# lutao98/SqrtLM-SLAM

Measured on AMD Instinct MI355X. Metric: LM iterations/sec (synthetic KITTI-00-scale BA), higher is better.
Workload: dtype f64; 1 GPU; synthetic global BA (BASELINE config 4); n_pose=5000, n_landmark=500000, n_obs=4999754, track_len=U{2..18}, robust=False, seed=4, parallelism=landmark-shard x1, comm=none, comm_ranks=1

## Files before the change

### include/sqrtlm.h

```cpp
#ifndef SQRTLM_H
#define SQRTLM_H

#include <stdint.h>

#ifdef __cplusplus
extern "C" {
#endif

#define SQLM_OK 0
#define SQLM_ERR_INVALID_ARG (-1)
#define SQLM_ERR_HIP (-2)
#define SQLM_ERR_NOT_SPD (-3)
#define SQLM_ERR_OOM (-4)
#define SQLM_ERR_ABORTED (-5)
#define SQLM_ERR_NO_DEVICE (-6)
#define SQLM_ERR_STATE (-7)
#define SQLM_ERR_UNSUPPORTED (-8)
#define SQLM_ERR_COMM (-9)

#define SQLM_TRACE_MAX 256

typedef struct sqlm_ctx sqlm_ctx;

typedef struct sqlm_stats {
// ... 225 lines not shown
#define SQLM_COMM_RCCL_SELFLOOP 2
#define SQLM_COMM_HOST 3
int sqlm_ctx_comm_info(const sqlm_ctx *ctx, int *transport, int *rank, int *nranks);
int sqlm_ctx_set_comm_selfloop(sqlm_ctx *ctx, const char *unique_id);
int sqlm_comm_selftest(int device, const char *unique_id, int64_t count, double *max_err);

#define SQLM_DT_F64 0
#define SQLM_DT_U8 1
#define SQLM_DT_I32 2
#define SQLM_OP_SUM 0
#define SQLM_OP_MAX 1
typedef int (*sqlm_allreduce_fn)(void *user, void *buf, int64_t count, int dtype, int op);
int sqlm_ctx_set_host_comm(sqlm_ctx *ctx, int rank, int nranks, sqlm_allreduce_fn fn, void *user);
#define SQLM_P2P_SEND 0
#define SQLM_P2P_RECV 1
#define SQLM_P2P_BCAST 2
typedef int (*sqlm_p2p_fn)(void *user, void *buf, int64_t count, int dtype, int peer, int op);
int sqlm_ctx_set_host_p2p(sqlm_ctx *ctx, sqlm_p2p_fn fn, void *user);

#define SQLM_NKERNEL_TIMERS 9
int sqlm_bench_iterations(sqlm_ctx *ctx, int warmup, int n, double *ms_per_iter, double *kernel_ms,
                          sqlm_stats *stats);
const char *sqlm_kernel_timer_name(int i);

#ifdef __cplusplus
}
#endif
#endif
```

### sqrtlm-slam_amd/csrc/sqlm_api.cpp

```cpp
#include <hip/hip_runtime.h>

#include <algorithm>
#include <cmath>
#include <cstring>
#include <new>
#include <vector>

#include "../../include/sqrtlm.h"
#include "../../include/sqrtlm_orb.h"
#include "se3_dev.h"
#include "sqlm_ctx.h"

using namespace sqlm;

namespace {

const char *kTimerNames[SQLM_NKERNEL_TIMERS] = {"k_linearize", "k_camera_pass", "k_damp", "k_rcs_tile",
                                                "k_solve", "k_pose_update", "k_landmark_update", "reduce+sync",
                                                "k_rcs_reduce"};

void depth_positive_host(const sqlm_ctx *c, std::vector<uint8_t> &out) {
  out.resize(c->n_obs);
  for (int64_t e = 0; e < c->n_obs; ++e) {
    const int p = c->obs_pose[e];
// ... 966 lines not shown
  s = comm_barrier(c->comm, c->stream);
  if (s) return s;
  c->timing = kernel_ms != nullptr;
  std::fill(c->kernel_ms_acc, c->kernel_ms_acc + SQLM_NKERNEL_TIMERS, 0.0);
  c->kernel_ms_n = 0;
  Timer t;
  s = run_lm(c, n, 0.0, nullptr, st, nullptr, true);
  SQLM_HIP_OK(hipStreamSynchronize(c->stream));
  const double ms = t.ms();
  c->timing = false;
  if (s) return s;
  if (ms_per_iter) *ms_per_iter = ms / n;
  if (kernel_ms) {
    for (int i = 0; i < SQLM_NKERNEL_TIMERS; ++i)
      kernel_ms[i] = c->kernel_ms_n ? c->kernel_ms_acc[i] / c->kernel_ms_n : 0.0;
  }
  return finish(c);
}

#ifdef SQLM_TILE_PROF
int sqlm_debug_tile_profile(long long *out) { return sqlm::tile_profile_read(out); }
#endif

const char *sqlm_kernel_timer_name(int i) {
  return (i >= 0 && i < SQLM_NKERNEL_TIMERS) ? kTimerNames[i] : "";
}

static int orb_engine(sqlm_ctx *c) {
  if (!c) return SQLM_ERR_INVALID_ARG;
  if (hipSetDevice(c->device) != hipSuccess) return SQLM_ERR_HIP;
  if (!c->orb && !(c->orb = orb_create(c->stream))) return SQLM_ERR_OOM;
  return SQLM_OK;
}

int sqlm_orb_extract(sqlm_ctx *c, const sqlm_orb_params *p, const uint8_t *image, int w, int h, int stride,
                     sqlm_keypoint *kps, uint8_t *desc, int cap, int *n_out) {
  if (int r = orb_engine(c)) return r;
  return orb_extract(c->orb, p, image, w, h, stride, kps, desc, cap, n_out);
}

int sqlm_orb_get_level(sqlm_ctx *c, int level, uint8_t *out, int cap, int *lw, int *lh) {
  if (!c || !c->orb) return SQLM_ERR_STATE;
  if (hipSetDevice(c->device) != hipSuccess) return SQLM_ERR_HIP;
  return orb_get_level(c->orb, level, out, cap, lw, lh);
}

// ... 82 lines not shown
```

### sqrtlm-slam_amd/csrc/sqlm_cr_aug.h

```cpp
#pragma once

namespace sqlm {
namespace aug {

#ifdef SQLM_AUG_SOLO
constexpr bool kPipe = false;
#else
constexpr bool kPipe = true;
#endif

constexpr int kWaves = 16, kThreads = 64 * kWaves, kMaxNt = kCRMaxN / 16, kWorkers = kPipe ? 10 : 12;
constexpr int kPairs = kMaxNt * (kMaxNt - 1) / 2;
enum : int { kNone = 0, kColD = 1, kColI0 = 3, kColEt = 4, kColE = 5, kColG = 6 };

#ifndef SQLM_SPIN_LIMIT
#define SQLM_SPIN_LIMIT (1 << 20)
#endif
constexpr int kSpinLimit = SQLM_SPIN_LIMIT;
constexpr int kTp = 17;
struct Shared {
  double T[kMaxNt][16 * kTp];
  double U[kPairs][256];
  double Hp[kMaxNt][256];
  double Hq[kMaxNt][256];
// ... 287 lines not shown
    if (q == 0) {
      sh.bx[16 * i + r] = x;
      st_d(v.x + (size_t)I * n + 16 * i + r, x);
    }
    __builtin_amdgcn_fence(__ATOMIC_RELEASE, "wavefront");
    __builtin_amdgcn_wave_barrier();
    __builtin_amdgcn_fence(__ATOMIC_ACQUIRE, "wavefront");
  }
}

constexpr int kCrErrTimeout = 1;
__device__ __forceinline__ void cr_fail(const CRView &v, int lane) {
  if (lane == 0) {
    __hip_atomic_store(v.flags, 0, __ATOMIC_RELAXED, __HIP_MEMORY_SCOPE_AGENT);
    __hip_atomic_store(v.flags + 1, kCrErrTimeout, __ATOMIC_RELAXED, __HIP_MEMORY_SCOPE_AGENT);
  }
}

template <int MODE, bool LINV, bool BACK>
__device__ __forceinline__ void aug_body(aug::Shared &sh, const CRView &v, int h, int I, int split, int sidx) {
  using namespace aug;
  const int lane = threadIdx.x & 63, wave = threadIdx.x >> 6;
  const int n = v.n, nt = n >> 4;
  const bool left = MODE == 0, right = MODE != 1 && I + h < v.p, first = sidx == 0;
  bool tmo = false;
  for (int t = threadIdx.x; t < 2 * kMaxNt + kPairs + 17; t += blockDim.x) {
    if (t < kMaxNt) sh.fT[t] = 0;
    else if (t < kMaxNt + kPairs) sh.fU[t - kMaxNt] = 0;
    else if (t < 2 * kMaxNt + kPairs) sh.fH[t - kMaxNt - kPairs] = 0;
    else if (t < 2 * kMaxNt + kPairs + 8) (&sh.fA[0][0])[t - 2 * kMaxNt - kPairs] = 0;
    else if (t < 2 * kMaxNt + kPairs + 16) (&sh.fO[0][0])[t - 2 * kMaxNt - kPairs - 8] = 0;
    else sh.fD = 0;
  }
  __syncthreads();
#ifdef SQLM_SPIN_DEBUG
  if (lane == 0 && (wave == 0 || wave == 9))
    printf("aug blk %d wave %d I %d mode %d past zeroing, fT0 %d\n", (int)blockIdx.x, wave, I, MODE, sh.fT[0]);
#endif
  if (threadIdx.x == 0) AUG_PROF(0);
  AUG_HWID(wave);
  const bool dense = MODE == 1 && v.ld;
  const int ldd = dense ? v.ld : n;
  const double *Dblk = dense ? v.D : blk(v.D, I, n);
  bool bad = false;
  if (kPipe && wave == 0) {
    __builtin_amdgcn_s_setprio(3);
    AUG_PROF(1);
// ... 284 lines not shown
```

### sqrtlm-slam_amd/csrc/sqlm_internal.h

```cpp
#pragma once
#include <hip/hip_runtime.h>
#include <stdint.h>

#include <cfloat>
#include <cmath>
#include <vector>

#include "../../include/sqrtlm.h"

namespace sqlm {

#define SQLM_HIP_OK(x)                          \
  do {                                          \
    if ((x) != hipSuccess) return SQLM_ERR_HIP; \
  } while (0)

#ifndef SQLM_TILE_MAXCAMS
#define SQLM_TILE_MAXCAMS 24
#endif
#ifndef SQLM_TILE_MAXLM
#define SQLM_TILE_MAXLM 128
#endif
constexpr int kTileMaxCams = SQLM_TILE_MAXCAMS, kTileHardCams = 24, kTileMaxLm = SQLM_TILE_MAXLM, kTileMaxK = 1 << 20;
constexpr int kTileNtMax = (6 * kTileHardCams + 15) / 16;
// ... 165 lines not shown
  int *flags = nullptr;
};

enum Scalar { kChiCur = 0, kChiNew = 1, kScale = 2, kMaxDiag = 3, kSolveOk = 4, kDevErr = 5, kNScalars = 8 };
constexpr int kMboxSeq = 7;

enum PartialRegion {
  kPartChiCurLm = 0,
  kPartChiCurLid = 16384,
  kPartChiNewLm = 147456,
  kPartChiNewLid = 163840,
  kPartScaleCam = 180224,
  kPartScaleLm = 196608,
  kPartChiCurLm2 = 212992,
  kPartChiCurLid2 = 229376,
  kPartEnd = 360448
};
constexpr int kMaxPartials = kPartEnd;
constexpr int kMaxFreePoses = 131072;

struct CRPlan {
  bool enabled = false;
  int B = 0, p = 0, n = 0;
  int nband = 0;
  int R = 0, Rp = 0, nbc = 0;
  std::vector<int> sched;
  const int *sched_dev = nullptr;
  std::vector<int> lvl;
  int init_off = 0, init_cnt = 0;
  int elim_off = 0, elim_cnt = 0;
  bool top_active = false;
};
constexpr int kCRMaxN = 112;
constexpr int kBandMaxCams = kCRMaxN / 6 - 1;
constexpr int kUpdHad = 1 << 28, kUpdRight = 1 << 29, kUpdLeft = 1 << 30, kUpdMask = (1 << 28) - 1;

__host__ __device__ inline int tile_blk(int u, int w, int cp) { return u * (2 * cp - u + 1) / 2 + (w - u); }

#ifndef SQLM_OBS_PER_LANE
#define SQLM_OBS_PER_LANE 3
#endif
constexpr int kObsPerLane = SQLM_OBS_PER_LANE;
#ifndef SQLM_OBS_PRELOAD
#define SQLM_OBS_PRELOAD 2
#endif
constexpr int kObsPreload = SQLM_OBS_PRELOAD;
// ... 34 lines not shown
void launch_rcs_tiles(const DevProblem &d, double lambda, hipStream_t st, const TileStreams *ts = nullptr);
enum TileKernel {
  kTileKernelNone = 0,
  kTileKernelRows = 1,
  kTileKernelMono = 2,
  kTileKernelStereo = 3,
  kTileKernelProducer = 4,
};
int rcs_tile_kernel(const DevProblem &d);
void launch_rcs_reduce(const DevProblem &d, double lambda, hipStream_t st);
#ifdef SQLM_TILE_PROF
int tile_profile_read(long long *out);
#endif
constexpr int kRedLong = 24;
int launch_dense_solve(const DevProblem &d, hipStream_t st);
struct CRSync {
  int *done = nullptr;
  int cap = 0, epoch = 0;
};
int launch_cr_solve(const DevProblem &d, const CRPlan &pl, hipStream_t st, bool gather = true,
                    CRSync *sync = nullptr);
void launch_arrow_clear(const DevProblem &d, const CRPlan &pl, hipStream_t st);
void launch_cr_core(double *D, double *L, double *E, double *A, double *C, double *g, double *x, int *flags, int p, int n,
                    hipStream_t st, CRSync *sync = nullptr);
int launch_dense_spd_solve(double *A, double *L, double *Linv, double *r, double *x, int *flags, int n,
                           hipStream_t st, int band = 0, int n_last = 0);
int launch_cr_multi(double *D, double *L, double *E, double *A, double *C, double *gs, double *xs, double *G, double *Z,
                    double *X, int *flags, int p, int n, int R, hipStream_t st);
int launch_batched_atb(const double *A, const double *B, double *P, int p, int n, int R, hipStream_t st);
void launch_pose_update(const DevProblem &d, double lambda, hipStream_t st, bool from_cr = false);
void launch_landmark_update(const DevProblem &d, const Bucket &b, double lambda, int part_off, hipStream_t st,
                            bool spec = false, bool fuse_pose = false);
constexpr int kMaxUpdBuckets = 6;
struct UpdLaunch {
  int nb = 0, grid = 0;
  int W[kMaxUpdBuckets], slot_begin[kMaxUpdBuckets], slot_end[kMaxUpdBuckets], part_off[kMaxUpdBuckets],
      rng_off[kMaxUpdBuckets], nblk[kMaxUpdBuckets], blk0[kMaxUpdBuckets];
};
int upd_launch_plan(const std::vector<Bucket> &bk, const std::vector<int> &part_off, UpdLaunch &u);
void launch_landmark_update_all(const DevProblem &d, const UpdLaunch &u, double lambda, hipStream_t st, bool spec);
void launch_lidar_chi2(const DevProblem &d, hipStream_t st);
void launch_reduce(const DevProblem &d, int n_lm_parts_cur, int n_lm_parts_new, int n_cam_parts,
                   int n_lid_parts, hipStream_t st, double *mbox = nullptr, unsigned long long seq = 0);
void launch_depth_positive(const DevProblem &d, uint8_t *out_dev, hipStream_t st);

int linearize_blocks(const Bucket &b);

// ... 350 lines not shown
```

### sqrtlm-slam_amd/csrc/sqlm_plan.cpp

```cpp
#include "sqlm_plan.h"

#include <limits>
#include <queue>

namespace sqlm {

void build_tiles(int nP, int nL, const std::vector<int> &lm_begin, const int *obs_camh, int lm_cap, TilePlan &tp,
                 TileBuild &tb, int *obs_local) {
  const int64_t nE = lm_begin[nL];
  PhaseTimer sub(kPhaseTiles);
  tp.reset();
  tp.urange.assign(nL, int2{-1, -1});
  std::vector<int> &tstart = tb.tstart;
  tstart.clear();
  {
    const int nchunk = (int)std::max<int64_t>(1, std::min<int64_t>(16, nE / 131072));
    const int nth = std::min(nchunk, host_threads(nE));
    std::vector<std::vector<int>> cuts(nchunk);
    std::vector<uint8_t> dup(nchunk, 0);
    run_threads(nth, [&](int th) {
      std::vector<int> stamp(nP, -1), lmst(nP, -1);
      for (int ch = th; ch < nchunk; ch += nth) {
        const int s0 = (int)((int64_t)nL * ch / nchunk), s1 = (int)((int64_t)nL * (ch + 1) / nchunk);
        std::vector<int> &cv = cuts[ch];
// ... 280 lines not shown
      }
      deg[v] = 0;
    }
  }
  const int nband = nP - nbc;
  if (nbc > 0) {
    if (nband == 0 || 3 * nbc > nP) return false;
    int pos = 0, b = 0;
    for (int i = 0; i < nP; ++i) cam_pos[i] = border[i] ? -1 - b++ : pos++;
  }
  int bw = 0;
  for (int i = 0; i < nP; ++i)
    for (int k = s_row[i]; k < s_row[i + 1]; ++k)
      if (cam_pos[i] >= 0 && cam_pos[s_col[k]] >= 0) bw = std::max(bw, cam_pos[s_col[k]] - cam_pos[i]);
  int B = std::min(bw + 1, std::max(nband, 1));
  if (nbc == 0) B = cr_superblock_width(B, nband);
  const int n = (6 * B + 15) / 16 * 16;
  if (n > kCRMaxN) return false;
  pl.enabled = true;
  pl.B = B;
  pl.p = (nband + B - 1) / B;
  pl.n = n;
  pl.nband = nband;
  if (nbc == 0) return true;
  pl.nbc = nbc;
  pl.R = (6 * nbc + 15) / 16 * 16;
  pl.Rp = (pl.R + kCRMaxN - 1) / kCRMaxN * kCRMaxN;
  std::vector<uint8_t> act(pl.p, 0);
  for (int i = 0; i < nP; ++i)
    for (int k = s_row[i]; k < s_row[i + 1]; ++k) {
      const int a = cam_pos[i], c2 = cam_pos[s_col[k]];
      if ((a < 0) != (c2 < 0)) act[(a >= 0 ? a : c2) / B] = 1;
    }
  std::vector<int> &S = pl.sched, elim;
  pl.init_off = 0;
  for (int I = 0; I < pl.p; ++I)
    if (act[I]) S.push_back(I);
  pl.init_cnt = (int)S.size();
  for (int h = 1; h < pl.p; h *= 2) {
    const int fo = (int)S.size();
    for (int I = h; I < pl.p; I += 2 * h)
      if (act[I]) { S.push_back(I); elim.push_back(I); }
    const int uo = (int)S.size();
    for (int J = 0; J < pl.p; J += 2 * h) {
      const bool r = J + h < pl.p && act[J + h], l = J >= h && act[J - h];
      if (!r && !l) continue;
      S.push_back(J | (act[J] ? kUpdHad : 0) | (r ? kUpdRight : 0) | (l ? kUpdLeft : 0));
// ... 508 lines not shown
```

### sqrtlm-slam_amd/csrc/sqlm_plan.h

```cpp
#pragma once
#include <cstdint>
#include <vector>

#include "sqlm_host_par.h"
#include "sqlm_internal.h"

namespace sqlm {

struct TilePlan {
  std::vector<int> lm_ptr{0}, cam_ptr{0}, cams, ld, red_ptr, gred_ptr;
  std::vector<int2> urange, gred_idx;
  std::vector<int64_t> red_off;
  std::vector<int64_t> gred_off;
  std::vector<int> long_s, long_g;
  std::vector<int64_t> part_ptr{0}, gpart_ptr{0};
  int max_cp = 0;
  bool dups = false;
  std::vector<int> order;
  int cls_off[kTileNtMax + 2] = {}, cls_cnt[kTileNtMax + 1] = {};
  void reset() {
    lm_ptr.assign(1, 0);
    cam_ptr.assign(1, 0);
    part_ptr.assign(1, 0);
    gpart_ptr.assign(1, 0);
// ... 2 lines not shown
    gred_idx.clear();
    red_off.clear();
    gred_off.clear();
    max_cp = 0;
    dups = false;
    std::fill(cls_off, cls_off + kTileNtMax + 2, 0);
    std::fill(cls_cnt, cls_cnt + kTileNtMax + 1, 0);
  }
};

struct TileBuild {
  struct Red { int key, tile, code, j; };
  struct TileOut { std::vector<int> cams; std::vector<Red> red; };
  std::vector<int> tstart;
  std::vector<TileOut> out;
};

void build_tiles(int nP, int nL, const std::vector<int> &lm_begin, const int *obs_camh, int lm_cap, TilePlan &tp,
                 TileBuild &tb, int *obs_local);
void pattern_from_tiles(int nP, const TileBuild &tb, std::vector<int> &s_row, std::vector<int> &s_col);
void build_tiles_finish(int nP, const std::vector<int> &s_row, const std::vector<int> &s_col, TilePlan &tp,
                        TileBuild &tb);
int cr_superblock_width(int bmin, int nband);
bool plan_rcs(int nP, const std::vector<int> &s_row, const std::vector<int> &s_col, CRPlan &pl,
              std::vector<int> &cam_pos);

inline int seg_width(int k) {
  int w = 2;
  while (kObsPerLane * w < k && w < 64) w <<= 1;
  return w;
}

struct GraphView {
  int n_pose = 0, n_pt = 0;
  int64_t n_obs = 0, n_lid = 0;
  const int32_t *obs_pose = nullptr, *obs_pt = nullptr;
  const double *obs_uv = nullptr, *obs_info = nullptr, *obs_delta = nullptr;
  const uint8_t *obs_level = nullptr;
  const double *obs_ur = nullptr;
  const uint8_t *pose_fixed = nullptr;
  const int32_t *lid_pose = nullptr;
  const double *lid_pc = nullptr, *lid_pw = nullptr, *lid_n = nullptr, *lid_info = nullptr;
  const uint8_t *lid_level = nullptr;
  const uint8_t *lid_kind = nullptr;
  int level = 0;
};
// ... 58 lines not shown
```

### sqrtlm-slam_amd/csrc/sqlm_rcs_solve.hip

```cpp
#include <hip/hip_runtime.h>

#include <algorithm>
#include <climits>
#include <cstdlib>

#include "sqlm_internal.h"

namespace sqlm {

typedef double d4 __attribute__((ext_vector_type(4)));

__device__ __forceinline__ void st_d(double *p, double v) { *p = v; }

#ifdef SQLM_CR_PROF
__device__ long long *g_cr_prof;
#define CR_PROF(i)                                                                    \
  do {                                                                                \
    if (threadIdx.x == 0 && g_cr_prof) g_cr_prof[blockIdx.x * 64 + (i)] = clock64(); \
  } while (0)
#else
#define CR_PROF(i) \
  do {             \
  } while (0)
#endif

__device__ __forceinline__ double readlane_d(double v, int l) {
  const int lo = __builtin_amdgcn_readlane(__double2loint(v), l);
  const int hi = __builtin_amdgcn_readlane(__double2hiint(v), l);
  return __hiloint2double(hi, lo);
// ... 233 lines not shown
        const int k = 4 * s + k4;
        a[4 * t + s] = t > jb ? L[(16 * jb + k) * ld + 16 * t + r16] : Dinv[jb * kTile + k * kT + r16];
        b[4 * t + s] = z[16 * t + k];
      }
    }
  double acc = 0.0;
#pragma unroll
  for (int t = 0; t < kCRMaxN / 16; ++t)
    if (t >= jb && t < nt) {
#pragma unroll
      for (int s = 0; s < 4; ++s) acc = fma(a[4 * t + s], b[4 * t + s], acc);
    }
  return k4_sum(acc);
}

struct CRView {
  int p, n, B, nP;
  double *D, *E, *A, *C, *g, *x;
  int *flags;
  double *L;
  int ld;
  int *done = nullptr;
  int epoch = 0;
};

__device__ __forceinline__ double *blk(double *base, int I, int n) { return base + (size_t)I * n * n; }

inline size_t cr_factor_lds(int n) { return ((size_t)n * (n + 1) + 37 * (size_t)n) * sizeof(double); }

__global__ __launch_bounds__(256) void k_cr_scatter(DevProblem d, CRView v) {
  const int i = blockIdx.x;
  const int n = v.n, R = d.arw_R, Rp = d.arw_Rp;
  const int pi = d.cam_pos ? d.cam_pos[i] : i;
  const int I = pi >= 0 ? pi / v.B : 0, li = pi >= 0 ? pi - I * v.B : 0;
  for (int s = d.s_row_ptr[i]; s < d.s_row_ptr[i + 1]; ++s) {
    const int j = d.s_col[s];
    const int pj = d.cam_pos ? d.cam_pos[j] : j;
    const int J = pj >= 0 ? pj / v.B : 0, lj = pj >= 0 ? pj - J * v.B : 0;
    for (int e = threadIdx.x; e < 36; e += blockDim.x) {
      const int r = e / 6, c = e % 6;
      const double val = d.S[(size_t)s * 36 + e];
      if (pi >= 0 && pj >= 0) {
        if (J == I) {
          blk(v.D, I, n)[(6 * li + r) * n + 6 * lj + c] = val;
          if (j != i) blk(v.D, I, n)[(6 * lj + c) * n + 6 * li + r] = val;
        } else {
// ... 212 lines not shown
  const int jobs = (I + h < v.p ? 2 : 1) * nt;
  const int q0 = sidx + split * wave, q1 = sidx + split * (wave + nw);
  double b0x[kCRMaxN / 8], b0y[kCRMaxN / 8], b1x[kCRMaxN / 8], b1y[kCRMaxN / 8];
  if (sidx == 0) cr_factor_store(v, I, lds, &fail);
  else cr_factor_block(v, I, lds, &fail);
  const double *L = lds, *Dinv = lds + n * ld + 2 * n;
  if (q0 < jobs) {
    if (q0 < nt) load_strip<true>(blk(v.E, I - h, n), n, q0, b0x, b0y);
    else load_strip<false>(blk(v.E, I, n), n, q0 - nt, b0x, b0y);
  }
  if (q1 < jobs) {
    if (q1 < nt) load_strip<true>(blk(v.E, I - h, n), n, q1, b1x, b1y);
    else load_strip<false>(blk(v.E, I, n), n, q1 - nt, b1x, b1y);
  }
  if (q0 < jobs) strip_tiles(L, ld, Dinv, b0x, b0y, q0 < nt ? blk(v.A, I, n) : blk(v.C, I, n), n, q0 % nt);
  if (q1 < jobs) strip_tiles(L, ld, Dinv, b1x, b1y, q1 < nt ? blk(v.A, I, n) : blk(v.C, I, n), n, q1 % nt);
}

inline int cr_split(int n_odd, int nt) { return std::max(1, std::min(2 * nt, 256 / std::max(1, n_odd))); }

__device__ __forceinline__ void cr_update_item(const CRView &v, int h, int lb) {
  const int n = v.n, nt = n >> 4, nd = nt * (nt + 1) / 2, items = nd + nt * nt + nt;
  const int ev = lb / items, rem = lb - ev * items;
  const int J = 2 * h * ev;
  const bool right = J + h < v.p, left = J >= h;
  const int lane = threadIdx.x & 63, r16 = lane & 15, k4 = lane >> 4;
  if (rem < nd) {
    int ti = 0, tj = rem;
    while (tj > ti) { tj -= ti + 1; ++ti; }
    d4 acc = {0.0, 0.0, 0.0, 0.0};
    if (right) acc = tile_gemm<true, false, false>(blk(v.A, J + h, n), blk(v.A, J + h, n), n, ti, tj);
    if (left) {
      const d4 a2 = tile_gemm<true, false, false>(blk(v.C, J - h, n), blk(v.C, J - h, n), n, ti, tj);
      acc += a2;
    }
    if (right || left) tile_store(blk(v.D, J, n), n, ti, tj, acc, -1.0, true);
  } else if (rem < nd + nt * nt) {
    const int t = rem - nd, ti = t / nt, tj = t - ti * nt;
    if (right && J + 2 * h < v.p) {
      const d4 acc = tile_gemm<true, false, false>(blk(v.A, J + h, n), blk(v.C, J + h, n), n, ti, tj);
      tile_store(blk(v.E, J, n), n, ti, tj, acc, -1.0, false);
    }
  } else {
    const int ar = 16 * (rem - nd - nt * nt) + r16;
    double s = 0.0;
    if (right) {
      const double *A = blk(v.A, J + h, n), *z = v.g + (size_t)(J + h) * n;
#pragma unroll
      for (int u = 0; u < kCRMaxN / 4; ++u) {
        const int k = kclamp(4 * u + k4, n);
        s += A[k * n + ar] * (4 * u < n ? z[k] : 0.0);
      }
    }
    if (left) {
      const double *C = blk(v.C, J - h, n), *z = v.g + (size_t)(J - h) * n;
#pragma unroll
      for (int u = 0; u < kCRMaxN / 4; ++u) {
        const int k = kclamp(4 * u + k4, n);
        s += C[k * n + ar] * (4 * u < n ? z[k] : 0.0);
      }
    }
    s = k4_sum(s);
// ... 17 lines not shown
  if (wave < nt) {
    const double s = linv_gemv(L, ld, Dinv, tmp, wave);
    if (k4 == 0) z[ar] = s;
  }
  __syncthreads();
  if (wave < nt) {
    const double s = linv_gemv_t(L, ld, Dinv, z, wave, nt);
    if (k4 == 0) v.x[ar] = s;
  }
  CR_PROF(34);
}

__global__ __launch_bounds__(512) void k_cr_top(CRView v) {
  extern __shared__ __attribute__((aligned(16))) double lds[];
  __shared__ int fail;
  cr_top_body(v, lds, &fail);
}

template <bool LINV>
__device__ __forceinline__ void cr_back_body(const CRView &v, int h, int I, double *t) {
  const int n = v.n;
  const int wave = threadIdx.x >> 6, lane = threadIdx.x & 63, lo = lane & 7, hi = lane >> 3;
  const bool act = wave < (n >> 4);
  const bool right = I + h < v.p;
  using d2 = HIP_vector_type<double, 2>;
  const int ca = 2 * lo;
  const d2 *A = reinterpret_cast<const d2 *>(blk(v.A, I, n)), *C = reinterpret_cast<const d2 *>(blk(v.C, I, n));
  const d2 *xl = reinterpret_cast<const d2 *>(v.x + (size_t)(I - h) * n);
  const d2 *xr = reinterpret_cast<const d2 *>(v.x + (size_t)(I + (right ? h : 0)) * n);
  const d2 *Li = reinterpret_cast<const d2 *>(blk(v.L, I, n));
  const int r0 = 16 * wave + hi, hn = n >> 1;
  d2 a0[kCRMaxN / 16], a1[kCRMaxN / 16], c0[kCRMaxN / 16], c1[kCRMaxN / 16], vl[kCRMaxN / 16], vr[kCRMaxN / 16];
  d2 li[kCRMaxN / 8];
  if (act) {
#pragma unroll
  for (int u = 0; u < kCRMaxN / 16; ++u) {
    const int c = kclamp(16 * u + ca, n) >> 1;
    a0[u] = A[r0 * hn + c];
    a1[u] = A[(r0 + 8) * hn + c];
    vl[u] = xl[c];
  }
  if (LINV) {
#pragma unroll
    for (int u = 0; u < kCRMaxN / 8; ++u) li[u] = Li[kclamp(16 * wave + 8 * u + hi, n) * hn + 8 * wave + lo];
  }
  if (right) {
#pragma unroll
    for (int u = 0; u < kCRMaxN / 16; ++u) {
      const int c = kclamp(16 * u + ca, n) >> 1;
      c0[u] = C[r0 * hn + c];
      c1[u] = C[(r0 + 8) * hn + c];
      vr[u] = xr[c];
    }
  }
  double s0 = 0.0, s1 = 0.0;
#pragma unroll
  for (int u = 0; u < kCRMaxN / 16; ++u)
    if (16 * u < n) {
      s0 += a0[u].x * vl[u].x + a0[u].y * vl[u].y;
      s1 += a1[u].x * vl[u].x + a1[u].y * vl[u].y;
      if (right) {
        s0 += c0[u].x * vr[u].x + c0[u].y * vr[u].y;
        s1 += c1[u].x * vr[u].x + c1[u].y * vr[u].y;
// ... 71 lines not shown
    }
  acc += __shfl_xor(acc, 16, 64);
  acc += __shfl_xor(acc, 32, 64);
  if (q == 0) rr[16 * i + r] = y[16 * i + r] - acc;
  __builtin_amdgcn_fence(__ATOMIC_RELEASE, "wavefront");
  __builtin_amdgcn_wave_barrier();
  __builtin_amdgcn_fence(__ATOMIC_ACQUIRE, "wavefront");
  double x = 0.0;
#pragma unroll
  for (int m = 0; m < 4; ++m) x = fma(tv[m], rr[16 * i + 4 * q + m], x);
  x += __shfl_xor(x, 16, 64);
  x += __shfl_xor(x, 32, 64);
  if (q == 0) {
    xs[16 * i + r] = x;
    st_d(v.x + (size_t)I * n + 16 * i + r, x);
  }
  aug::raise_flag(&fx[i], lane);
  if (tmo) cr_fail(v, lane);
}

template <bool TOP>
__global__ __launch_bounds__(512) void k_cr_back_u(CRView v, int h) {
  extern __shared__ __attribute__((aligned(16))) double sm[];
  back_u_body<TOP>(sm, v, h, TOP ? 0 : h + 2 * h * blockIdx.x);
}

__device__ __forceinline__ bool wait_x(const CRView &v, int J) {
  bool ok = J == 0;
  const int *f = v.done + J;
  for (int it = 0; !ok && it < aug::kSpinLimit; ++it) {
    if (__hip_atomic_load(f, __ATOMIC_RELAXED, __HIP_MEMORY_SCOPE_AGENT) == v.epoch) ok = true;
    else __builtin_amdgcn_s_sleep(2);
  }
#ifdef SQLM_SPIN_FORCE_TIMEOUT
  ok = false;
#endif
  return ok;
}
__device__ __forceinline__ double ld_x(const double *p) {
  return __hip_atomic_load(p, __ATOMIC_RELAXED, __HIP_MEMORY_SCOPE_AGENT);
}

__device__ __forceinline__ void back_all_body(double *sm, const CRView &v, int h, int I) {
  double *y = sm, *rr = sm + kCRMaxN, *xs = sm + 2 * kCRMaxN;
  int *fx = reinterpret_cast<int *>(sm + 3 * kCRMaxN);
  __shared__ int tmo_s;
  const int n = v.n, nt = n >> 4;
  const int wave = threadIdx.x >> 6, lane = threadIdx.x & 63, q = lane >> 4, r = lane & 15;
  const int lo = lane & 7, hi = lane >> 3;
  const bool right = I + h < v.p;
  if (threadIdx.x < aug::kMaxNt) fx[threadIdx.x] = 0;
  const int i = wave;
  const double *Lb = blk(v.L, I, n);
  double u[aug::kMaxNt][4], tv[4];
#pragma unroll
  for (int j = 0; j < aug::kMaxNt; ++j)
    if (j > i && j < nt) {
#pragma unroll
      for (int m = 0; m < 4; ++m) u[j][m] = Lb[(size_t)(16 * i + r) * n + 16 * j + 4 * q + m];
    }
#pragma unroll
  for (int m = 0; m < 4; ++m) tv[m] = Lb[(size_t)(16 * i + 4 * q + m) * n + 16 * i + r];
  using d2 = HIP_vector_type<double, 2>;
  const int ca = 2 * lo;
  const d2 *A = reinterpret_cast<const d2 *>(blk(v.A, I, n)), *C = reinterpret_cast<const d2 *>(blk(v.C, I, n));
  const int r0 = 16 * wave + hi, hn = n >> 1;
  d2 a0[kCRMaxN / 16], a1[kCRMaxN / 16], c0[kCRMaxN / 16], c1[kCRMaxN / 16];
#pragma unroll
  for (int uu = 0; uu < kCRMaxN / 16; ++uu) {
    const int c = kclamp(16 * uu + ca, n) >> 1;
    a0[uu] = A[r0 * hn + c];
    a1[uu] = A[(r0 + 8) * hn + c];
  }
  if (right) {
#pragma unroll
    for (int uu = 0; uu < kCRMaxN / 16; ++uu) {
      const int c = kclamp(16 * uu + ca, n) >> 1;
      c0[uu] = C[r0 * hn + c];
      c1[uu] = C[(r0 + 8) * hn + c];
    }
  }
  const double z0 = v.g[(size_t)I * n + r0], z1 = v.g[(size_t)I * n + r0 + 8];
  if (threadIdx.x == 0) {
    bool ok = wait_x(v, I - h);
    if (right) ok = wait_x(v, I + h) && ok;
    tmo_s = ok ? 0 : 1;
  }
  __syncthreads();
  const bool tmo = tmo_s != 0;
  const double *xl = v.x + (size_t)(I - h) * n, *xr = v.x + (size_t)(I + (right ? h : 0)) * n;
  d2 vl[kCRMaxN / 16], vr[kCRMaxN / 16];
#pragma unroll
  for (int uu = 0; uu < kCRMaxN / 16; ++uu) {
    const int c = (kclamp(16 * uu + ca, n) >> 1) << 1;
    vl[uu].x = ld_x(xl + c);
    vl[uu].y = ld_x(xl + c + 1);
    if (right) {
      vr[uu].x = ld_x(xr + c);
      vr[uu].y = ld_x(xr + c + 1);
    }
  }
  double s0 = 0.0, s1 = 0.0;
#pragma unroll
  for (int uu = 0; uu < kCRMaxN / 16; ++uu)
    if (16 * uu < n) {
      s0 += a0[uu].x * vl[uu].x + a0[uu].y * vl[uu].y;
      s1 += a1[uu].x * vl[uu].x + a1[uu].y * vl[uu].y;
      if (right) {
        s0 += c0[uu].x * vr[uu].x + c0[uu].y * vr[uu].y;
        s1 += c1[uu].x * vr[uu].x + c1[uu].y * vr[uu].y;
      }
    }
#pragma unroll
  for (int m = 1; m < 8; m <<= 1) {
    s0 += __shfl_xor(s0, m, 64);
    s1 += __shfl_xor(s1, m, 64);
  }
  if (lo == 0) {
    y[r0] = z0 - s0;
// ... 15 lines not shown
  __builtin_amdgcn_fence(__ATOMIC_RELEASE, "wavefront");
  __builtin_amdgcn_wave_barrier();
  __builtin_amdgcn_fence(__ATOMIC_ACQUIRE, "wavefront");
  double x = 0.0;
#pragma unroll
  for (int m = 0; m < 4; ++m) x = fma(tv[m], rr[16 * i + 4 * q + m], x);
  x += __shfl_xor(x, 16, 64);
  x += __shfl_xor(x, 32, 64);
  if (q == 0) {
    xs[16 * i + r] = x;
    __hip_atomic_store(v.x + (size_t)I * n + 16 * i + r, x, __ATOMIC_RELAXED, __HIP_MEMORY_SCOPE_AGENT);
  }
  aug::raise_flag(&fx[i], lane);
  if (tmo || tw) cr_fail(v, lane);
  asm volatile("s_waitcnt vmcnt(0)" ::: "memory");
  __syncthreads();
  if (threadIdx.x == 0) __hip_atomic_store(v.done + I, v.epoch, __ATOMIC_RELAXED, __HIP_MEMORY_SCOPE_AGENT);
}

__global__ __launch_bounds__(512) void k_cr_back_all(CRView v, int h_top) {
  extern __shared__ __attribute__((aligned(16))) double sm[];
  int b = blockIdx.x, h = h_top;
  for (;;) {
    const int n_odd = (v.p - h + 2 * h - 1) / (2 * h);
    if (b < n_odd || h == 1) break;
    b -= n_odd;
    h >>= 1;
  }
  back_all_body(sm, v, h, h + 2 * h * b);
}


struct DenseView {
  int n, nblk;
  double *A, *L, *Linv;
  double *r, *x;
  int *flags;
};

__global__ __launch_bounds__(512) void k_dchol_diag(DenseView v, int k, int nk) {
  extern __shared__ __attribute__((aligned(16))) double lds[];
  __shared__ int fail;
  constexpr int nb = kCRMaxN;
  const int ld = nb + 1, nw = blockDim.x >> 6, wave = threadIdx.x >> 6, lane = threadIdx.x & 63;
  double *L = lds, *tmp = lds + nb * ld, *Dinv = tmp + 2 * nb, *W = Dinv + 17 * nb, *invd = W + 17 * nb;
  const double *Ak = v.A + (size_t)k * nb * v.n + (size_t)k * nb;
  for (int r = wave; r < nk; r += nw)
// ... 331 lines not shown
  const int rt = R >> 4, per = rt * rt, I = lb / per, t = lb - I * per, ti = t / rt, tj = t - ti * rt;
  const size_t nr = (size_t)n * R;
  const d4 acc = mm_tile<true>(A + I * nr, R, B + I * nr, R, ti, tj, 0, n);
  mm_store(P + (size_t)I * R * R, R, ti, tj, acc, 1.0, false);
}

int launch_batched_atb(const double *A, const double *B, double *P, int p, int n, int R, hipStream_t st) {
  if (p <= 0 || n % 4 || R % 16) return -1;
  const int total = p * (R / 16) * (R / 16);
  hipLaunchKernelGGL(k_batched_atb, dim3(xcd_grid(total)), dim3(64), 0, st, A, B, P, n, R, total);
  return hipGetLastError() == hipSuccess ? 0 : -2;
}

__global__ __launch_bounds__(512) void k_cr_factor_at(CRView v, int I) {
  extern __shared__ __attribute__((aligned(16))) double lds[];
  __shared__ int fail;
  cr_factor_store(v, I, lds, &fail);
}

__device__ __forceinline__ void trsm_strip(const CRView &v, int h, int I, int s) {
  const int n = v.n, nt = n >> 4, lane = threadIdx.x & 63, b = lane >> 4, i16 = lane & 15;
  const bool et = s < nt;
  const int J = et ? s : s - nt;
  if (!et && I + h >= v.p) return;
  const double *Lb = blk(v.L, I, n);
  d4 t[aug::kMaxNt];
#pragma unroll
  for (int r = 0; r < aug::kMaxNt; ++r)
    if (r < nt)
      t[r] = et ? aug::load_tile_t(blk(v.E, I - h, n), n, 16 * r, 16 * J, lane)
                : aug::load_tile(blk(v.E, I, n), n, 16 * r, 16 * J, lane);
  double ta[4];
  d4 u[aug::kMaxNt];
  auto load_step = [&](int k, double (&a)[4], d4 (&uu)[aug::kMaxNt]) {
#pragma unroll
    for (int m = 0; m < 4; ++m) a[m] = Lb[(size_t)(16 * k + i16) * n + 16 * k + 4 * m + b];
#pragma unroll
    for (int r = 1; r < aug::kMaxNt; ++r)
      if (r > k && r < nt) uu[r] = aug::load_tile(Lb, n, 16 * k, 16 * r, lane);
  };
  load_step(0, ta, u);
#pragma unroll
  for (int k = 0; k < aug::kMaxNt; ++k) {
    if (k >= nt) break;
    double ta_n[4];
    d4 u_n[aug::kMaxNt];
    if (k + 1 < nt) load_step(k + 1, ta_n, u_n);
// ... 266 lines not shown
    }
    const int ncr = n_even * upd, tot = ncr + uc * rhs;
    hipLaunchKernelGGL(k_arw_update_gemm, dim3(xcd_grid(tot)), dim3(64), 0, st, v, a, h, ncr, S + uo, tot);
  }
  launch_cr_factor(v, 0, 0, 0, 1, true, st);
  const int *elim = S + pl.elim_off;
  if (pl.top_active)
    hipLaunchKernelGGL(k_arw_fwd, dim3(xcd_grid(rhs)), dim3(64), 0, st, a, elim + pl.elim_cnt - 1, rhs);
  if (pl.elim_cnt) {
    const int rt = R / 16, lt = rt * (rt + 1) / 2;
    hipLaunchKernelGGL(k_arw_gram, dim3(xcd_grid(lt)), dim3(64), 0, st, a, elim, pl.elim_cnt, d.bd_A, pl.Rp, lt);
    hipLaunchKernelGGL(k_arw_gvec, dim3(R / 16), dim3(64), 0, st, a, elim, pl.elim_cnt, d.bd_r);
  }
  launch_dense_spd_solve(d.bd_A, d.bd_L, d.bd_Linv, d.bd_r, d.bd_x, d.flags, pl.Rp, st, 0, R - (pl.Rp - kCRMaxN));
  if (pl.elim_cnt)
    hipLaunchKernelGGL(k_arw_correct, dim3((pl.elim_cnt * n + 3) / 4), dim3(256), 0, st, a, elim, pl.elim_cnt, d.bd_x);
  hipLaunchKernelGGL(k_arw_top_back, dim3(1), dim3(512), 0, st, a, d.cr_x);
  for (h /= 2; h >= 1; h /= 2) {
    const int n_odd = (p - h + 2 * h - 1) / (2 * h);
    hipLaunchKernelGGL(k_cr_back, dim3(n_odd), dim3(64 * nt), (size_t)n * sizeof(double), st, v, h);
  }
}

void launch_cr_core(double *D, double *L, double *E, double *A, double *C, double *g, double *x, int *flags, int p,
                    int n, hipStream_t st, CRSync *sync) {
  CRView v{p, n, 0, 0, D, E, A, C, g, x, flags, L};
  const size_t lds = cr_factor_lds(n);
  const int nt = n / 16, per = nt * nt, upd = nt * (nt + 1) / 2 + per + nt;
  int h = 1;
  for (; h < p; h *= 2) {
    const int n_odd = (p - h + 2 * h - 1) / (2 * h);
    const int n_even = (p + 2 * h - 1) / (2 * h);
    launch_cr_level(v, h, n_odd, false, st);
    hipLaunchKernelGGL(k_cr_update_gemm, dim3(xcd_grid(n_even * upd)), dim3(64), 0, st, v, h, n_even * upd);
  }
  const size_t back_lds = 3 * kCRMaxN * sizeof(double) + aug::kMaxNt * sizeof(int);
  if (cr_legacy())
    hipLaunchKernelGGL(k_cr_top, dim3(1), dim3(512), lds, st, v);
  else
    hipLaunchKernelGGL((k_cr_aug<1, false, true>), dim3(1), dim3(aug::kThreads), sizeof(aug::Shared), st, v, 0, 0, 0, 1);
  if (!cr_legacy() && p > 1 && sync && sync->done && sync->cap >= p) {
    if (sync->epoch == INT_MAX) {
      (void)hipMemsetAsync(sync->done, 0, (size_t)sync->cap * sizeof(int), st);
      sync->epoch = 0;
    }
    v.done = sync->done;
    v.epoch = ++sync->epoch;
    hipLaunchKernelGGL(k_cr_back_all, dim3(p - 1), dim3(64 * nt), back_lds, st, v, h / 2);
    return;
  }
  for (h /= 2; h >= 1; h /= 2) {
    const int n_odd = (p - h + 2 * h - 1) / (2 * h);
    if (cr_legacy())
      hipLaunchKernelGGL(k_cr_back, dim3(n_odd), dim3(64 * nt), (size_t)n * sizeof(double), st, v, h);
    else
      hipLaunchKernelGGL(k_cr_back_u<false>, dim3(n_odd), dim3(64 * nt), back_lds, st, v, h);
  }
}

int launch_cr_solve(const DevProblem &d, const CRPlan &pl, hipStream_t st, bool gather, CRSync *sync) {
  CRView v{pl.p, pl.n, pl.B, d.nP, d.cr_D, d.cr_E, d.cr_A, d.cr_C, d.cr_g, d.cr_x, d.flags, d.cr_L};
  if (!d.cr_direct) {
    const size_t blkbytes = (size_t)pl.p * pl.n * pl.n * sizeof(double);
    if (hipMemsetAsync(d.cr_D, 0, blkbytes, st) != hipSuccess) return -2;
    if (hipMemsetAsync(d.cr_E, 0, blkbytes, st) != hipSuccess) return -2;
    if (pl.R) launch_arrow_clear(d, pl, st);
    hipLaunchKernelGGL(k_cr_scatter, dim3(d.nP), dim3(64), 0, st, d, v);
  }
  if (pl.R) launch_arrow_solve(d, pl, st);
  else launch_cr_core(d.cr_D, d.cr_L, d.cr_E, d.cr_A, d.cr_C, d.cr_g, d.cr_x, d.flags, pl.p, pl.n, st, sync);
  if (gather) hipLaunchKernelGGL(k_cr_gather, dim3((6 * d.nP + 255) / 256), dim3(256), 0, st, d, v);
  return 0;
}

}
```

### sqrtlm-slam_amd/sqrtlm/_lib.py

```python
from __future__ import annotations

import ctypes as C
import os

import numpy as np

_HERE = os.path.dirname(os.path.abspath(__file__))
LIB_PATH = os.environ.get("SQLM_LIB_PATH", os.path.join(_HERE, "libsqrtlm.so"))
TRACE_MAX = 256
NKERNEL_TIMERS = 9

SQLM_OK = 0
STATUS = {0: "ok", -1: "invalid argument", -2: "HIP runtime error", -3: "not SPD", -4: "out of device memory",
          -5: "aborted", -6: "no HIP device", -7: "state error", -8: "unsupported problem shape", -9: "RCCL error"}

EXPORTS = [
    "sqlm_version", "sqlm_status_string", "sqlm_ctx_create", "sqlm_ctx_destroy", "sqlm_set_problem",
    "sqlm_set_lidar", "sqlm_set_edge_level", "sqlm_set_robust", "sqlm_set_lidar_level", "sqlm_optimize",
    "sqlm_local_ba", "sqlm_global_ba", "sqlm_get_poses", "sqlm_get_points", "sqlm_get_edge_chi2",
    "sqlm_get_edge_depth_positive", "sqlm_get_edge_level", "sqlm_pose_from_Tcw_f32", "sqlm_pose_to_Tcw_f32",
    "sqlm_comm_id_size", "sqlm_comm_get_unique_id", "sqlm_ctx_set_comm", "sqlm_ctx_set_host_comm",
    "sqlm_ctx_set_host_p2p", "sqlm_ctx_set_comm_selfloop", "sqlm_comm_selftest", "sqlm_ctx_comm_info",
    "sqlm_bench_iterations",
    "sqlm_kernel_timer_name", "sqlm_set_stereo",
    "sqlm_eg_set_problem", "sqlm_eg_optimize", "sqlm_eg_get_poses", "sqlm_eg_get_edge_chi2",
    "sqlm_eg_get_jacobians", "sqlm_eg_get_last_step", "sqlm_eg_get_exec_info",
    "sqlm_get_rcs_layout", "sqlm_get_exec_info", "sqlm_get_last_step",
    "sqlm_sim3_optimize", "sqlm_sim3_get_pair_chi2", "sqlm_sim3_get_linearization", "sqlm_sim3_get_last_step",
    "sqlm_pose_optimize", "sqlm_pose_refine_lidar", "sqlm_pose_get_edge_chi2", "sqlm_pose_get_linearization",
    "sqlm_pose_get_last_step",
    "sqlm_lidar_associate", "sqlm_set_lidar_from_clouds", "sqlm_lidar_get_exec_info",
    "sqlm_get_lidar_error",
    "sqlm_set_lidar_kind", "sqlm_set_lidar_from_cloud_sets",
    "sqlm_sim3_ransac", "sqlm_sim3_ransac_get_inliers", "sqlm_sim3_ransac_get_hypothesis",
    "sqlm_sim3_ransac_max_its", "sqlm_sim3_ransac_scan", "sqlm_sim3_ransac_hypothesis_host",
    "sqlm_pnp_ransac", "sqlm_pnp_ransac_get_inliers", "sqlm_pnp_ransac_get_refined", "sqlm_pnp_ransac_get_hypothesis",
    "sqlm_pnp_ransac_max_its", "sqlm_pnp_ransac_scan", "sqlm_pnp_ransac_hypothesis_host",
    "sqlm_pnp_ransac_refine_host",
]
CAPTURE_EXPORTS = ["sqlm_capture_write", "sqlm_capture_read", "sqlm_capture_free", "sqlm_capture_replay",
                   "sqlm_save_trajectory_kitti"]
ORB_EXPORTS = ["sqlm_orb_extract", "sqlm_orb_get_level", "sqlm_orb_match_bf", "sqlm_orb_search_for_init",
               "sqlm_orb_search_by_projection_local", "sqlm_orb_search_by_projection_last",
               "sqlm_orb_search_by_projection_sim3", "sqlm_orb_fuse", "sqlm_orb_search_by_projection_kf",
               "sqlm_orb_search_by_sim3", "sqlm_orb_search_by_bow_kf_frame", "sqlm_orb_search_by_bow_kf_kf", "sqlm_orb_search_for_triangulation",
               "sqlm_orb_bench_extract",
               "sqlm_voc_create", "sqlm_voc_destroy", "sqlm_voc_info", "sqlm_bow_transform", "sqlm_bow_score",
# ... 155 lines not shown
```

Baseline: 595.7 LM iterations/s.

## Offset cyclic-reduction block indexing so the reduction tree ends at a power of two

Adds a base offset lo to the block-tridiagonal cyclic reduction, defaulting to one for plans without arrow columns. Block I is addressed as I-lo, the top block becomes a power of two, and left/right boundary checks are generalised. A precomputed level table drives the forward, update and backward launches. The aim is to change the level count and per-level odd/even block counts to cut wasted boundary work or launches. It adds a debug export and a SQLM_CR_LO0 escape hatch, and the pointer-offset indexing is a correctness risk.

```diff
diff --git a/include/sqrtlm.h b/include/sqrtlm.h
--- a/include/sqrtlm.h
+++ b/include/sqrtlm.h
@@ -271,6 +271,7 @@
 int sqlm_bench_iterations(sqlm_ctx *ctx, int warmup, int n, double *ms_per_iter, double *kernel_ms,
                           sqlm_stats *stats);
 const char *sqlm_kernel_timer_name(int i);
+int sqlm_debug_cr_levels(int out[3]);
 
 #ifdef __cplusplus
 }
diff --git a/sqrtlm-slam_amd/csrc/sqlm_api.cpp b/sqrtlm-slam_amd/csrc/sqlm_api.cpp
--- a/sqrtlm-slam_amd/csrc/sqlm_api.cpp
+++ b/sqrtlm-slam_amd/csrc/sqlm_api.cpp
@@ -1012,6 +1012,12 @@
 int sqlm_debug_tile_profile(long long *out) { return sqlm::tile_profile_read(out); }
 #endif
 
+int sqlm_debug_cr_levels(int out[3]) {
+  if (!out) return SQLM_ERR_INVALID_ARG;
+  sqlm::cr_last_levels(out);
+  return SQLM_OK;
+}
+
 const char *sqlm_kernel_timer_name(int i) {
   return (i >= 0 && i < SQLM_NKERNEL_TIMERS) ? kTimerNames[i] : "";
 }
diff --git a/sqrtlm-slam_amd/csrc/sqlm_cr_aug.h b/sqrtlm-slam_amd/csrc/sqlm_cr_aug.h
--- a/sqrtlm-slam_amd/csrc/sqlm_cr_aug.h
+++ b/sqrtlm-slam_amd/csrc/sqlm_cr_aug.h
@@ -333,7 +333,7 @@
   using namespace aug;
   const int lane = threadIdx.x & 63, wave = threadIdx.x >> 6;
   const int n = v.n, nt = n >> 4;
-  const bool left = MODE == 0, right = MODE != 1 && I + h < v.p, first = sidx == 0;
+  const bool left = MODE == 0 && I - h >= v.lo, right = MODE != 1 && I + h < v.p + v.lo, first = sidx == 0;
   bool tmo = false;
   for (int t = threadIdx.x; t < 2 * kMaxNt + kPairs + 17; t += blockDim.x) {
     if (t < kMaxNt) sh.fT[t] = 0;
diff --git a/sqrtlm-slam_amd/csrc/sqlm_internal.h b/sqrtlm-slam_amd/csrc/sqlm_internal.h
--- a/sqrtlm-slam_amd/csrc/sqlm_internal.h
+++ b/sqrtlm-slam_amd/csrc/sqlm_internal.h
@@ -211,6 +211,7 @@
 struct CRPlan {
   bool enabled = false;
   int B = 0, p = 0, n = 0;
+  int lo = 0;
   int nband = 0;
   int R = 0, Rp = 0, nbc = 0;
   std::vector<int> sched;
@@ -291,7 +292,8 @@
                     CRSync *sync = nullptr);
 void launch_arrow_clear(const DevProblem &d, const CRPlan &pl, hipStream_t st);
 void launch_cr_core(double *D, double *L, double *E, double *A, double *C, double *g, double *x, int *flags, int p, int n,
-                    hipStream_t st, CRSync *sync = nullptr);
+                    hipStream_t st, CRSync *sync = nullptr, int lo = 0);
+void cr_last_levels(int out[3]);
 int launch_dense_spd_solve(double *A, double *L, double *Linv, double *r, double *x, int *flags, int n,
                            hipStream_t st, int band = 0, int n_last = 0);
 int launch_cr_multi(double *D, double *L, double *E, double *A, double *C, double *gs, double *xs, double *G, double *Z,
diff --git a/sqrtlm-slam_amd/csrc/sqlm_plan.cpp b/sqrtlm-slam_amd/csrc/sqlm_plan.cpp
--- a/sqrtlm-slam_amd/csrc/sqlm_plan.cpp
+++ b/sqrtlm-slam_amd/csrc/sqlm_plan.cpp
@@ -326,7 +326,10 @@
   pl.p = (nband + B - 1) / B;
   pl.n = n;
   pl.nband = nband;
-  if (nbc == 0) return true;
+  if (nbc == 0) {
+    pl.lo = std::getenv("SQLM_CR_LO0") ? 0 : 1;
+    return true;
+  }
   pl.nbc = nbc;
   pl.R = (6 * nbc + 15) / 16 * 16;
   pl.Rp = (pl.R + kCRMaxN - 1) / kCRMaxN * kCRMaxN;
diff --git a/sqrtlm-slam_amd/csrc/sqlm_plan.h b/sqrtlm-slam_amd/csrc/sqlm_plan.h
--- a/sqrtlm-slam_amd/csrc/sqlm_plan.h
+++ b/sqrtlm-slam_amd/csrc/sqlm_plan.h
@@ -48,6 +48,32 @@
 void build_tiles_finish(int nP, const std::vector<int> &s_row, const std::vector<int> &s_col, TilePlan &tp,
                         TileBuild &tb);
 int cr_superblock_width(int bmin, int nband);
+
+struct CRLevels {
+  static constexpr int kMax = 32;
+  int lo = 0, top = 0, count = 0, back_grid = 0;
+  int h[kMax] = {}, n_odd[kMax] = {}, n_even[kMax] = {};
+};
+inline CRLevels cr_levels(int p, int lo) {
+  CRLevels L;
+  L.lo = lo;
+  const int last = p + lo - 1;
+  int h = 1;
+  for (; L.count < CRLevels::kMax && last / h + 1 - lo >= 2; h *= 2) {
+    L.h[L.count] = h;
+    L.n_odd[L.count] = (last + h) / (2 * h);
+    L.n_even[L.count] = last / (2 * h) + 1 - lo;
+    L.back_grid += L.n_odd[L.count];
+    ++L.count;
+  }
+  L.top = lo ? h : 0;
+  return L;
+}
+inline void cr_back_block(const CRLevels &L, int b, int &level, int &I) {
+  level = L.count - 1;
+  while (level > 0 && b >= L.n_odd[level]) b -= L.n_odd[level--];
+  I = L.h[level] + 2 * L.h[level] * b;
+}
 bool plan_rcs(int nP, const std::vector<int> &s_row, const std::vector<int> &s_col, CRPlan &pl,
               std::vector<int> &cam_pos);
 
diff --git a/sqrtlm-slam_amd/csrc/sqlm_rcs_solve.hip b/sqrtlm-slam_amd/csrc/sqlm_rcs_solve.hip
--- a/sqrtlm-slam_amd/csrc/sqlm_rcs_solve.hip
+++ b/sqrtlm-slam_amd/csrc/sqlm_rcs_solve.hip
@@ -1,10 +1,12 @@
 #include <hip/hip_runtime.h>
 
 #include <algorithm>
+#include <atomic>
 #include <climits>
 #include <cstdlib>
 
 #include "sqlm_internal.h"
+#include "sqlm_plan.h"
 
 namespace sqlm {
 
@@ -284,6 +286,7 @@
   int ld;
   int *done = nullptr;
   int epoch = 0;
+  int lo = 0, top = 0;
 };
 
 __device__ __forceinline__ double *blk(double *base, int I, int n) { return base + (size_t)I * n * n; }
@@ -542,8 +545,8 @@
 __device__ __forceinline__ void cr_update_item(const CRView &v, int h, int lb) {
   const int n = v.n, nt = n >> 4, nd = nt * (nt + 1) / 2, items = nd + nt * nt + nt;
   const int ev = lb / items, rem = lb - ev * items;
-  const int J = 2 * h * ev;
-  const bool right = J + h < v.p, left = J >= h;
+  const int J = 2 * h * (ev + v.lo), pe = v.p + v.lo;
+  const bool right = J + h < pe, left = J - h >= v.lo;
   const int lane = threadIdx.x & 63, r16 = lane & 15, k4 = lane >> 4;
   if (rem < nd) {
     int ti = 0, tj = rem;
@@ -557,7 +560,7 @@
     if (right || left) tile_store(blk(v.D, J, n), n, ti, tj, acc, -1.0, true);
   } else if (rem < nd + nt * nt) {
     const int t = rem - nd, ti = t / nt, tj = t - ti * nt;
-    if (right && J + 2 * h < v.p) {
+    if (right && J + 2 * h < pe) {
       const d4 acc = tile_gemm<true, false, false>(blk(v.A, J + h, n), blk(v.C, J + h, n), n, ti, tj);
       tile_store(blk(v.E, J, n), n, ti, tj, acc, -1.0, false);
     }
@@ -621,11 +624,11 @@
   const int n = v.n;
   const int wave = threadIdx.x >> 6, lane = threadIdx.x & 63, lo = lane & 7, hi = lane >> 3;
   const bool act = wave < (n >> 4);
-  const bool right = I + h < v.p;
+  const bool right = I + h < v.p + v.lo, left = I - h >= v.lo;
   using d2 = HIP_vector_type<double, 2>;
   const int ca = 2 * lo;
   const d2 *A = reinterpret_cast<const d2 *>(blk(v.A, I, n)), *C = reinterpret_cast<const d2 *>(blk(v.C, I, n));
-  const d2 *xl = reinterpret_cast<const d2 *>(v.x + (size_t)(I - h) * n);
+  const d2 *xl = reinterpret_cast<const d2 *>(v.x + (size_t)(I - (left ? h : 0)) * n);
   const d2 *xr = reinterpret_cast<const d2 *>(v.x + (size_t)(I + (right ? h : 0)) * n);
   const d2 *Li = reinterpret_cast<const d2 *>(blk(v.L, I, n));
   const int r0 = 16 * wave + hi, hn = n >> 1;
@@ -635,9 +638,9 @@
 #pragma unroll
   for (int u = 0; u < kCRMaxN / 16; ++u) {
     const int c = kclamp(16 * u + ca, n) >> 1;
-    a0[u] = A[r0 * hn + c];
-    a1[u] = A[(r0 + 8) * hn + c];
-    vl[u] = xl[c];
+    a0[u] = left ? A[r0 * hn + c] : d2(0.0, 0.0);
+    a1[u] = left ? A[(r0 + 8) * hn + c] : d2(0.0, 0.0);
+    vl[u] = left ? xl[c] : d2(0.0, 0.0);
   }
   if (LINV) {
 #pragma unroll
@@ -755,11 +758,11 @@
 template <bool TOP>
 __global__ __launch_bounds__(512) void k_cr_back_u(CRView v, int h) {
   extern __shared__ __attribute__((aligned(16))) double sm[];
-  back_u_body<TOP>(sm, v, h, TOP ? 0 : h + 2 * h * blockIdx.x);
+  back_u_body<TOP>(sm, v, h, TOP ? v.top : h + 2 * h * blockIdx.x);
 }
 
 __device__ __forceinline__ bool wait_x(const CRView &v, int J) {
-  bool ok = J == 0;
+  bool ok = J == v.top;
   const int *f = v.done + J;
   for (int it = 0; !ok && it < aug::kSpinLimit; ++it) {
     if (__hip_atomic_load(f, __ATOMIC_RELAXED, __HIP_MEMORY_SCOPE_AGENT) == v.epoch) ok = true;
@@ -781,7 +784,7 @@
   const int n = v.n, nt = n >> 4;
   const int wave = threadIdx.x >> 6, lane = threadIdx.x & 63, q = lane >> 4, r = lane & 15;
   const int lo = lane & 7, hi = lane >> 3;
-  const bool right = I + h < v.p;
+  const bool right = I + h < v.p + v.lo, left = I - h >= v.lo;
   if (threadIdx.x < aug::kMaxNt) fx[threadIdx.x] = 0;
   const int i = wave;
   const double *Lb = blk(v.L, I, n);
@@ -802,8 +805,8 @@
 #pragma unroll
   for (int uu = 0; uu < kCRMaxN / 16; ++uu) {
     const int c = kclamp(16 * uu + ca, n) >> 1;
-    a0[uu] = A[r0 * hn + c];
-    a1[uu] = A[(r0 + 8) * hn + c];
+    a0[uu] = left ? A[r0 * hn + c] : d2(0.0, 0.0);
+    a1[uu] = left ? A[(r0 + 8) * hn + c] : d2(0.0, 0.0);
   }
   if (right) {
 #pragma unroll
@@ -815,19 +818,20 @@
   }
   const double z0 = v.g[(size_t)I * n + r0], z1 = v.g[(size_t)I * n + r0 + 8];
   if (threadIdx.x == 0) {
-    bool ok = wait_x(v, I - h);
+    bool ok = true;
+    if (left) ok = wait_x(v, I - h);
     if (right) ok = wait_x(v, I + h) && ok;
     tmo_s = ok ? 0 : 1;
   }
   __syncthreads();
   const bool tmo = tmo_s != 0;
-  const double *xl = v.x + (size_t)(I - h) * n, *xr = v.x + (size_t)(I + (right ? h : 0)) * n;
+  const double *xl = v.x + (size_t)(I - (left ? h : 0)) * n, *xr = v.x + (size_t)(I + (right ? h : 0)) * n;
   d2 vl[kCRMaxN / 16], vr[kCRMaxN / 16];
 #pragma unroll
   for (int uu = 0; uu < kCRMaxN / 16; ++uu) {
     const int c = (kclamp(16 * uu + ca, n) >> 1) << 1;
-    vl[uu].x = ld_x(xl + c);
-    vl[uu].y = ld_x(xl + c + 1);
+    vl[uu].x = left ? ld_x(xl + c) : 0.0;
+    vl[uu].y = left ? ld_x(xl + c + 1) : 0.0;
     if (right) {
       vr[uu].x = ld_x(xr + c);
       vr[uu].y = ld_x(xr + c + 1);
@@ -889,7 +893,7 @@
   extern __shared__ __attribute__((aligned(16))) double sm[];
   int b = blockIdx.x, h = h_top;
   for (;;) {
-    const int n_odd = (v.p - h + 2 * h - 1) / (2 * h);
+    const int n_odd = (v.p + v.lo - 1 + h) / (2 * h);
     if (b < n_odd || h == 1) break;
     b -= n_odd;
     h >>= 1;
@@ -1267,7 +1271,7 @@
   const int n = v.n, nt = n >> 4, lane = threadIdx.x & 63, b = lane >> 4, i16 = lane & 15;
   const bool et = s < nt;
   const int J = et ? s : s - nt;
-  if (!et && I + h >= v.p) return;
+  if (et ? I - h < v.lo : I + h >= v.p + v.lo) return;
   const double *Lb = blk(v.L, I, n);
   d4 t[aug::kMaxNt];
 #pragma unroll
@@ -1580,39 +1584,49 @@
   }
 }
 
+static std::atomic<int> g_cr_last[3];
+void cr_last_levels(int out[3]) {
+  for (int i = 0; i < 3; ++i) out[i] = g_cr_last[i].load();
+}
+
 void launch_cr_core(double *D, double *L, double *E, double *A, double *C, double *g, double *x, int *flags, int p,
-                    int n, hipStream_t st, CRSync *sync) {
-  CRView v{p, n, 0, 0, D, E, A, C, g, x, flags, L};
+                    int n, hipStream_t st, CRSync *sync, int lo) {
+  if (cr_legacy()) lo = 0;
+  const CRLevels lv = cr_levels(p, lo);
+  g_cr_last[0] = lo;
+  g_cr_last[1] = lv.count;
+  g_cr_last[2] = lv.top;
+  const size_t nn = (size_t)n * n;
+  CRView v{p, n, 0, 0, D - lo * nn, E - lo * nn, A - lo * nn, C - lo * nn, g - lo * n, x - lo * n, flags, L - lo * nn};
+  v.lo = lo;
+  v.top = lv.top;
   const size_t lds = cr_factor_lds(n);
   const int nt = n / 16, per = nt * nt, upd = nt * (nt + 1) / 2 + per + nt;
-  int h = 1;
-  for (; h < p; h *= 2) {
-    const int n_odd = (p - h + 2 * h - 1) / (2 * h);
-    const int n_even = (p + 2 * h - 1) / (2 * h);
-    launch_cr_level(v, h, n_odd, false, st);
-    hipLaunchKernelGGL(k_cr_update_gemm, dim3(xcd_grid(n_even * upd)), dim3(64), 0, st, v, h, n_even * upd);
+  for (int l = 0; l < lv.count; ++l) {
+    const int h = lv.h[l];
+    launch_cr_level(v, h, lv.n_odd[l], false, st);
+    hipLaunchKernelGGL(k_cr_update_gemm, dim3(xcd_grid(lv.n_even[l] * upd)), dim3(64), 0, st, v, h, lv.n_even[l] * upd);
   }
   const size_t back_lds = 3 * kCRMaxN * sizeof(double) + aug::kMaxNt * sizeof(int);
   if (cr_legacy())
     hipLaunchKernelGGL(k_cr_top, dim3(1), dim3(512), lds, st, v);
   else
-    hipLaunchKernelGGL((k_cr_aug<1, false, true>), dim3(1), dim3(aug::kThreads), sizeof(aug::Shared), st, v, 0, 0, 0, 1);
-  if (!cr_legacy() && p > 1 && sync && sync->done && sync->cap >= p) {
+    hipLaunchKernelGGL((k_cr_aug<1, false, true>), dim3(1), dim3(aug::kThreads), sizeof(aug::Shared), st, v, 0, v.top, 0, 1);
+  if (!cr_legacy() && lv.count > 0 && sync && sync->done && sync->cap >= p) {
     if (sync->epoch == INT_MAX) {
       (void)hipMemsetAsync(sync->done, 0, (size_t)sync->cap * sizeof(int), st);
       sync->epoch = 0;
     }
-    v.done = sync->done;
+    v.done = sync->done - lo;
     v.epoch = ++sync->epoch;
-    hipLaunchKernelGGL(k_cr_back_all, dim3(p - 1), dim3(64 * nt), back_lds, st, v, h / 2);
+    hipLaunchKernelGGL(k_cr_back_all, dim3(lv.back_grid), dim3(64 * nt), back_lds, st, v, lv.h[lv.count - 1]);
     return;
   }
-  for (h /= 2; h >= 1; h /= 2) {
-    const int n_odd = (p - h + 2 * h - 1) / (2 * h);
+  for (int l = lv.count - 1; l >= 0; --l) {
     if (cr_legacy())
-      hipLaunchKernelGGL(k_cr_back, dim3(n_odd), dim3(64 * nt), (size_t)n * sizeof(double), st, v, h);
+      hipLaunchKernelGGL(k_cr_back, dim3(lv.n_odd[l]), dim3(64 * nt), (size_t)n * sizeof(double), st, v, lv.h[l]);
     else
-      hipLaunchKernelGGL(k_cr_back_u<false>, dim3(n_odd), dim3(64 * nt), back_lds, st, v, h);
+      hipLaunchKernelGGL(k_cr_back_u<false>, dim3(lv.n_odd[l]), dim3(64 * nt), back_lds, st, v, lv.h[l]);
   }
 }
 
@@ -1626,7 +1640,7 @@
     hipLaunchKernelGGL(k_cr_scatter, dim3(d.nP), dim3(64), 0, st, d, v);
   }
   if (pl.R) launch_arrow_solve(d, pl, st);
-  else launch_cr_core(d.cr_D, d.cr_L, d.cr_E, d.cr_A, d.cr_C, d.cr_g, d.cr_x, d.flags, pl.p, pl.n, st, sync);
+  else launch_cr_core(d.cr_D, d.cr_L, d.cr_E, d.cr_A, d.cr_C, d.cr_g, d.cr_x, d.flags, pl.p, pl.n, st, sync, pl.lo);
   if (gather) hipLaunchKernelGGL(k_cr_gather, dim3((6 * d.nP + 255) / 256), dim3(256), 0, st, d, v);
   return 0;
 }
diff --git a/sqrtlm-slam_amd/sqrtlm/_lib.py b/sqrtlm-slam_amd/sqrtlm/_lib.py
--- a/sqrtlm-slam_amd/sqrtlm/_lib.py
+++ b/sqrtlm-slam_amd/sqrtlm/_lib.py
@@ -22,7 +22,7 @@
     "sqlm_comm_id_size", "sqlm_comm_get_unique_id", "sqlm_ctx_set_comm", "sqlm_ctx_set_host_comm",
     "sqlm_ctx_set_host_p2p", "sqlm_ctx_set_comm_selfloop", "sqlm_comm_selftest", "sqlm_ctx_comm_info",
     "sqlm_bench_iterations",
-    "sqlm_kernel_timer_name", "sqlm_set_stereo",
+    "sqlm_kernel_timer_name", "sqlm_debug_cr_levels", "sqlm_set_stereo",
     "sqlm_eg_set_problem", "sqlm_eg_optimize", "sqlm_eg_get_poses", "sqlm_eg_get_edge_chi2",
     "sqlm_eg_get_jacobians", "sqlm_eg_get_last_step", "sqlm_eg_get_exec_info",
     "sqlm_get_rcs_layout", "sqlm_get_exec_info", "sqlm_get_last_step",
```

Result: faster. 619.6 LM iterations/s (median of 6 runs) (+4.0%).
